# MaartenGr/ReinLife

Measured on AMD Instinct MI355X. Metric: agent-steps/sec (env.step + policy fwd), 30x30 grid, 100 agents, higher is better.
Workload: dtype f32-grade policy via block-scaled 2 x f16 split on v_mfma_f32_32x32x16_f16 (f32 accumulate) / int32+u8 world state / f64 rewards

## Files before the change

### reinlife_amd/csrc/rl_policy_dev.h

```cpp
#pragma once
#include "rl_common.h"

namespace {

typedef float f32x16 __attribute__((ext_vector_type(16)));
typedef float f32x4 __attribute__((ext_vector_type(4)));
typedef float f32x4u __attribute__((ext_vector_type(4), aligned(4)));
typedef float f32x2 __attribute__((ext_vector_type(2)));
typedef _Float16 f16x8 __attribute__((ext_vector_type(8)));
typedef const float __attribute__((address_space(1))) gfloat;
typedef const f32x4 __attribute__((address_space(1))) gf32x4;

constexpr int kInChunks = 10;
constexpr int kPlanes = 2;
constexpr int kScaleExp = 10;

__host__ __device__ constexpr int64_t frag_floats(int chunks, int tout) { return (int64_t)chunks * tout * kPlanes * 64 * 4; }
__host__ __device__ constexpr int64_t in_layer_floats(int tout) { return frag_floats(kInChunks, tout) + (int64_t)tout * 64; }
__host__ __device__ constexpr int64_t hid_layer_floats(int tin, int tout) { return frag_floats(2 * tin, tout) + (int64_t)tout * 64; }
__host__ __device__ constexpr int64_t head_consts_off(int tin) { return frag_floats(2 * tin, 1); }
__host__ __device__ constexpr int64_t head_floats(int tin, int nout) { return head_consts_off(tin) + 16; }

struct Layout {
    int64_t l1, l2a, l2b, ha, hb, total;
// ... 464 lines not shown
        a1 = mfma16(ac[1][0], B[S][1], a1); __builtin_amdgcn_sched_barrier(0);
    }
    a0 = mfma16(ac[0][0], B[S][0], a0); shadow(IntC<S>{}, IntC<0>{}, IntC<4 * S + 0>{}); __builtin_amdgcn_sched_barrier(0);
    a1 = mfma16(ac[1][0], B[S][0], a1); shadow(IntC<S>{}, IntC<1>{}, IntC<4 * S + 1>{}); __builtin_amdgcn_sched_barrier(0);
    a0 = mfma16(ac[0][1], B[S][0], a0); shadow(IntC<S>{}, IntC<2>{}, IntC<4 * S + 2>{}); __builtin_amdgcn_sched_barrier(0);
    a1 = mfma16(ac[1][1], B[S][0], a1); shadow(IntC<S>{}, IntC<3>{}, IntC<4 * S + 3>{}); __builtin_amdgcn_sched_barrier(0);
    if constexpr (S + 1 < kInChunks) k_pass_inx_steps<HALF, XM, S + 1>(w, B, a0, a1, shadow);
}
template <int HALF, int XM, typename Ring, typename Shadow>
__device__ __forceinline__ void k_pass_inx(Ring& w, const f32x4 (&B)[kInChunks][kPlanes], f32x16& a0, f32x16& a1, Shadow&& shadow)
{
#pragma unroll
    for (int r = 0; r < 16; ++r) { a0[r] = 0.0f; a1[r] = 0.0f; }
    k_pass_inx_steps<HALF, XM, 0>(w, B, a0, a1, shadow);
}
template <int XM, int C, int K, typename Raw>
__device__ __forceinline__ void in_split_slot(Raw&& raw, float sc, f32x4& hi, f32x4& lo)
{
    constexpr int cls = in_chunk_class(C);
    { float v; split_hi(raw(2 * K), raw(2 * K + 1), sc, v); hi[K] = v; }
    if constexpr (K == 1 || K == 3) {
        if constexpr (!(cls != 0 && XM >= cls)) {
            float v;
            split_lo(raw(2 * K - 2), raw(2 * K - 1), sc, hi[K - 1], v); lo[K - 1] = v;
            split_lo(raw(2 * K), raw(2 * K + 1), sc, hi[K], v); lo[K] = v;
        }
    }
}

template <int NS, int HALF, typename Ring, typename Shadow>
__device__ inline void k_pass(Ring& w, const f32x4 (&B)[NS][kPlanes], f32x16& a0, f32x16& a1, Shadow&& shadow)
{
#pragma unroll
    for (int r = 0; r < 16; ++r) { a0[r] = 0.0f; a1[r] = 0.0f; }
#pragma unroll
    for (int s = 0; s < NS; ++s) {
        f32x4 ac[2][kPlanes];
        w.take(HALF * NS + s, ac);
        a0 = mfma16(ac[0][0], B[s][1], a0); shadow(6 * s + 0); __builtin_amdgcn_sched_barrier(0);
        a1 = mfma16(ac[1][0], B[s][1], a1); shadow(6 * s + 1); __builtin_amdgcn_sched_barrier(0);
        a0 = mfma16(ac[0][0], B[s][0], a0); shadow(6 * s + 2); __builtin_amdgcn_sched_barrier(0);
        a1 = mfma16(ac[1][0], B[s][0], a1); shadow(6 * s + 3); __builtin_amdgcn_sched_barrier(0);
        a0 = mfma16(ac[0][1], B[s][0], a0); shadow(6 * s + 4); __builtin_amdgcn_sched_barrier(0);
        a1 = mfma16(ac[1][1], B[s][0], a1); shadow(6 * s + 5); __builtin_amdgcn_sched_barrier(0);
    }
}

__device__ inline void max3_abs(float& m, float a, float b)
{
#if defined(__HIP_DEVICE_COMPILE__)
    asm("v_max3_f32 %0, %0, |%1|, |%2|" : "+v"(m) : "v"(a), "v"(b));
#endif
}

struct EpiStream {
    const float* c;
    f32x4 un[2], bi[2];
    __device__ inline void fetch(int t, int Q)
    {
        const float* q = c + (t + (Q >> 2)) * 64 + 4 * (Q & 3);
        un[Q & 1] = *(const f32x4*)q;
        bi[Q & 1] = *(const f32x4*)(q + 16);
    }
    __device__ inline void step(int t, int e, f32x16& a0, f32x16& a1, float row_un, float& m)
    {
        const int Q = e >> 2, r = e & 15, ee = e & 3;
        if (ee == 0 && Q + 1 < 8) fetch(t, Q + 1);
        f32x16& a = e < 16 ? a0 : a1;
        const float y = fmaxf(__builtin_fmaf(a[r], un[Q & 1][ee] * row_un, bi[Q & 1][ee]), 0.0f);
        a[r] = y;
        m = fmaxf(m, y);
    }
};

template <int D, int NCH = 8, typename Raw>
__device__ inline void head_stream(WRing<1, 1, 1, D>& w, const f32x4& un4, Raw&& raw, float sc, float row_un, float (&out)[4])
{
    f32x16 a0, a1, a2;
#pragma unroll
    for (int r = 0; r < 16; ++r) { a0[r] = 0.0f; a1[r] = 0.0f; a2[r] = 0.0f; }
    f32x4 B[NCH][kPlanes];
#pragma unroll
    for (int k = 0; k < 3; ++k) split_slice<3>(k, [&](int e) { return raw(0, e); }, sc, B[0][0], B[0][1]);
#pragma unroll
    for (int s = 0; s < NCH; ++s) {
        f32x4 ac[1][kPlanes];
        w.template next<NCH>(s, ac);
        a0 = mfma16(ac[0][0], B[s][1], a0);
        if (s + 1 < NCH) split_slice<3>(0, [&](int e) { return raw(s + 1, e); }, sc, B[(s + 1) % NCH][0], B[(s + 1) % NCH][1]);
        __builtin_amdgcn_sched_barrier(0);
        a1 = mfma16(ac[0][0], B[s][0], a1);
        if (s + 1 < NCH) split_slice<3>(1, [&](int e) { return raw(s + 1, e); }, sc, B[(s + 1) % NCH][0], B[(s + 1) % NCH][1]);
        __builtin_amdgcn_sched_barrier(0);
        a2 = mfma16(ac[0][1], B[s][0], a2);
        if (s + 1 < NCH) split_slice<3>(2, [&](int e) { return raw(s + 1, e); }, sc, B[(s + 1) % NCH][0], B[(s + 1) % NCH][1]);
        __builtin_amdgcn_sched_barrier(0);
    }
#pragma unroll
    for (int r = 0; r < 4; ++r) out[r] = ((a0[r] + a1[r]) + a2[r]) * (un4[r] * row_un);
}

struct PairLds {
    float* pmax;
    f32x4* ex;
    float* val;
};
struct Tile1Part {
    float head[4];
    rl_u4 draw;
};

#ifndef RL_CERT_COUNT
#define RL_CERT_COUNT(greedy_mask, cert_mask, fell_back) do { } while (0)
#endif
template <int KIND>
__device__ __attribute__((noinline, cold)) void tile1_cert_fallback(TileIO io, const f32x4* ex, float un1, f32x4 adv4, rl_u4 draw)
{
    extern __shared__ __attribute__((aligned(16))) char rl_dyn_lds[];
    constexpr int D = 3;
    const int lane = (int)__builtin_amdgcn_mbcnt_hi(~0u, __builtin_amdgcn_mbcnt_lo(~0u, 0u)), h = lane >> 5;
    const Layout L = layout_of(KIND);
    const float* const consts = (const float*)(rl_dyn_lds + io.c_lds_off) + 32 * h;
    const float* const hconsts = (const float*)(rl_dyn_lds + io.c_lds_off) + 768;
    WRingH<8, D> w;
    w.start(io.packed + L.l2b, lane);
    f32x4 B2[8][kPlanes];
#pragma unroll
    for (int c = 0; c < 8; ++c)
#pragma unroll
        for (int pl = 0; pl < kPlanes; ++pl) B2[c][pl] = ex[(c * kPlanes + pl) * 64 + lane];
    f32x16 A[4];
    EpiStream ep;
    float mrow = 0.0f;
    k_pass<8, 0>(w, B2, A[0], A[1], [&](int) {});
    ep.c = consts + 512;
    k_pass<8, 1>(w, B2, A[2], A[3], [&](int slot) {
        if (slot == 0) ep.fetch(0, 0);
        if (slot >= 2 && slot < 34) ep.step(0, slot - 2, A[0], A[1], un1, mrow);
    });
    WRing<1, 1, 1, D> wh;
    wh.start(io.packed + L.hb, lane, 0);
    ep.fetch(2, 0);
#pragma unroll
    for (int e = 0; e < 32; ++e) ep.step(2, e, A[2], A[3], un1, mrow);
    mrow = fmaxf(mrow, __shfl_xor(mrow, 32));
    float sc2, un2;
    row_scale(mrow, sc2, un2);
    auto araw = [&](int c, int e) { return A[c >> 1][8 * (c & 1) + e]; };
    float val[4];
    head_stream<D>(wh, *(const f32x4*)(hconsts + 16 + 4 * h), araw, sc2, un2, val);
    const float adv[4] = {adv4.x, adv4.y, adv4.z, adv4.w};
    tile1_finish<KIND>(io, lane, adv, val[0] + hconsts[16 + 8], draw, *(const f32x4*)(hconsts + 8 + 4 * h));
}
template <int KIND>
__device__ inline void tile1_finish_cert(const TileIO& io, int lane, const float (&adv)[4], const rl_u4& draw, const float* hconsts, float vbar,
                                         const f32x4* ex, float un1)
{
    const int h = lane >> 5;
    const f32x4 ba = *(const f32x4*)(hconsts + 8 + 4 * h);
    const float a4[4] = {adv[0] + ba.x, adv[1] + ba.y, adv[2] + ba.z, adv[3] + ba.w};
    float o4[4];
#pragma unroll
    for (int r = 0; r < 4; ++r) o4[r] = __shfl_xor(a4[r], 32);
    int act = 0;
    bool greedy = false, ok = true;
    if (h == 0) {
        const float a[8] = {a4[0], a4[1], a4[2], a4[3], o4[0], o4[1], o4[2], o4[3]};
        float best = a[0], amax = fabsf(a[0]), s = a[0];
        int is = 0;
#pragma unroll
        for (int i = 1; i < 8; ++i) {
            const bool gt = a[i] > best;
            is = gt ? i : is; best = gt ? a[i] : best;
            amax = fmaxf(amax, fabsf(a[i])); s += a[i];
        }
        const float thr = 0x1p-20f * (((amax + amax) + vbar) + 0x1p-80f) + (s - s);
#pragma unroll
        for (int j = 0; j < 7; ++j) ok = ok && (j >= is || best - a[j] > thr);
        const bool explore = (float)rl_u24(draw.x) < io.eps;
        act = explore ? (int)(draw.y >> 29) : is;
        greedy = io.valid && io.actions && !explore;
    }
    const bool need = greedy && !ok;
    RL_CERT_COUNT(__ballot(greedy), __ballot(greedy && ok), __any(need));
    if (__builtin_expect(__any(need), 0)) {
        tile1_cert_fallback<KIND>(io, ex, un1, f32x4{adv[0], adv[1], adv[2], adv[3]}, draw);
        return;
    }
    if (h == 0 && io.valid && io.actions) {
        io.actions[io.row] = (int8_t)act;
        if (io.lds_actions_off >= 0) {
            extern __shared__ __attribute__((aligned(16))) char rl_dyn_lds[];
            ((signed char*)rl_dyn_lds)[io.lds_actions_off + io.lds_slot] = (signed char)act;
        }
    }
}

__device__ inline void cert_bound_part(gfloat* __restrict__ pk, int tid, double& c0, double& c1)
{
    const Layout L = layout_of(RL_PERD3QN);
    const int t2 = tid >> 7, pl = (tid >> 6) & 1, lane = tid & 63, oo = lane & 31, o = 32 * t2 + oo;
    const int h = (oo >> 2) & 1, r = (oo & 3) + 4 * (oo >> 3);
    gf32x4* f = (gf32x4*)(pk + L.l2b) + (t2 * kPlanes + pl) * 64 + lane;
    f32x4 u[8];
#pragma unroll
    for (int s = 0; s < 8; ++s) u[s] = f[s * 4 * kPlanes * 64];
    const float un_o = pk[L.l2b + frag_floats(8, 4) + (t2 * 2 + h) * 32 + r], b1 = pk[L.l2b + frag_floats(8, 4) + (t2 * 2 + h) * 32 + 16 + r];
    typedef const _Float16 __attribute__((address_space(1))) gf16;
    gf16* hw = (gf16*)(pk + L.hb);
    const int hidx = (((o >> 5) * 2 + (r >> 3)) * kPlanes * 64 + 32 * h) * 8 + (r & 7);
    const double w = (double)fabsf((float)hw[hidx]) + (double)fabsf((float)hw[hidx + 64 * 8]);
    const double un_v = (double)pk[L.hb + head_consts_off(4)];
    double sum = 0.0;
#pragma unroll
    for (int s = 0; s < 8; ++s) {
        const f16x8 v = __builtin_bit_cast(f16x8, u[s]);
#pragma unroll
        for (int e = 0; e < 8; ++e) sum += (double)fabsf((float)v[e]);
    }
    const double wv = w * un_v;
    c1 = wv * (sum * (double)un_o);
    c0 = (pl == 0 && lane < 32) ? wv * (double)fabsf(b1) : 0.0;
}
__device__ inline float f32_up(double d)
{
    float f = (float)d;
    if ((double)f < d) f = __builtin_bit_cast(float, __builtin_bit_cast(unsigned, f) + (f >= 0.0f ? 1u : -1u));
    return f;
}

template <int KIND, bool COHERENT, bool PAIR = false, int XM = 0, bool CERT = false>
__device__ inline void policy_tile1s(const TileIO& io, int lane, int role = 0, const PairLds* pair_lds = nullptr, Tile1Part* part = nullptr)
{
    static_assert(KIND == RL_D3QN || KIND == RL_PERD3QN, "one-wave tile: dueling kinds");
    static_assert(!CERT || PAIR, "the certified argmax: the pair tile");
    extern __shared__ __attribute__((aligned(16))) char rl_dyn_lds[];
    constexpr int D = 3;
    const int h = lane >> 5;
    const Layout L = layout_of(KIND);
    gfloat* __restrict__ packed = io.packed;
    const float* const consts = (const float*)(rl_dyn_lds + io.c_lds_off) + 32 * h;
    const float* const hconsts = (const float*)(rl_dyn_lds + io.c_lds_off) + 768;
    RL_PMARK1(1);
    WRingH<kInChunks, D, PAIR ? kInChunks : 2 * kInChunks> w1;
    w1.start(packed + L.l1 + (PAIR ? role * (2 * kPlanes * 64 * 4) : 0), lane);
    f32x4 X[kInChunks][2];
    {
        const int64_t rbase = io.row * RL_OBS_DIM;
        if (io.x_lds_off >= 0) {
            const float* xr = (const float*)(rl_dyn_lds + io.x_lds_off);
#pragma unroll
            for (int c = 0; c < kInChunks; ++c)
#pragma unroll
                for (int q = 0; q < 2; ++q) {
                    if (c == kInChunks - 1 && h == 1) X[c][q] = f32x4{xr[149], xr[150], xr[151], xr[152]};
                    else X[c][q] = *(const f32x4*)(xr + 16 * c + 8 * h + 4 * q);
                }
        } else
#pragma unroll
        for (int c = 0; c < kInChunks; ++c)
#pragma unroll
            for (int q = 0; q < 2; ++q) {
                const int k0 = (c == kInChunks - 1 && h == 1) ? 149 : 16 * c + 8 * h + 4 * q;
                if (COHERENT) {
                    const __amdgpu_buffer_rsrc_t rsrc = __builtin_amdgcn_make_buffer_rsrc((void*)io.obs, 0, 0x7fffffff, 0x00027000);
                    X[c][q] = __builtin_bit_cast(f32x4, __builtin_amdgcn_raw_buffer_load_b128(rsrc, (int)((rbase + k0) * 4), 0, 16 ));
                } else
                    X[c][q] = *(const f32x4u*)(io.obs + rbase + k0);
            }
    }
    rl_u4 draw = {0u, 0u, 0u, 0u};
    if ((!PAIR || role == 0) && io.actions && io.eps > 0.0f) draw = rl_philox4x32(io.seed, io.key_epoch, io.key_world, io.key_tick, RL_SITE_ACT, io.key_index);
    if (h == 1) { X[kInChunks - 1][0] = f32x4{X[kInChunks - 1][0].w, 0.0f, 0.0f, 0.0f}; X[kInChunks - 1][1] = f32x4{0.0f, 0.0f, 0.0f, 0.0f}; }
    float sc0, un0;
    if constexpr (XM >= 1) row_scale(1.0f, sc0, un0);
    else {
        float m4[4] = {0.0f, 0.0f, 0.0f, 0.0f};
#pragma unroll
        for (int c = 0; c < kInChunks; ++c)
#pragma unroll
            for (int q = 0; q < 2; ++q) {
                max3_abs(m4[(2 * c + q) & 3], X[c][q].x, X[c][q].y);
                max3_abs(m4[(2 * c + q + 2) & 3], X[c][q].z, X[c][q].w);
            }
        float m = fmaxf(fmaxf(m4[0], m4[1]), fmaxf(m4[2], m4[3]));
        m = fmaxf(m, __shfl_xor(m, 32));
        row_scale(m, sc0, un0);
    }
    f32x4 B1[kInChunks][kPlanes];
    auto xraw = [&](int c, int e) { return X[c][e >> 2][e & 3]; };
    f32x16 F[4];
    EpiStream ep;
    if constexpr (XM >= 1) {
        auto x0 = [&](int e) { return xraw(0, e); };
        in_split_slot<XM, 0, 0>(x0, sc0, B1[0][0], B1[0][1]); in_split_slot<XM, 0, 1>(x0, sc0, B1[0][0], B1[0][1]);
        in_split_slot<XM, 0, 2>(x0, sc0, B1[0][0], B1[0][1]); in_split_slot<XM, 0, 3>(x0, sc0, B1[0][0], B1[0][1]);
        RL_PMARK1(2);
        k_pass_inx<0, XM>(w1, B1, F[0], F[1], [&](auto st, auto k, auto) {
            constexpr int c = decltype(st)::value + 1;
            if constexpr (c < kInChunks) in_split_slot<XM, c, decltype(k)::value>([&](int e) { return xraw(c, e); }, sc0, B1[c][0], B1[c][1]);
        });
    } else {
#pragma unroll
        for (int k = 0; k < 6; ++k) split_slice<6>(k, [&](int e) { return xraw(0, e); }, sc0, B1[0][0], B1[0][1]);
        RL_PMARK1(2);
        k_pass<kInChunks, 0>(w1, B1, F[0], F[1], [&](int slot) {
            const int c = slot / 6 + 1;
            if (c < kInChunks) split_slice<6>(slot % 6, [&](int e) { return xraw(c, e); }, sc0, B1[c][0], B1[c][1]);
        });
    }
    float mrow = 0.0f;
    const int64_t l2 = (PAIR && role) ? L.l2b : L.l2a, hd = (PAIR && role) ? L.hb : L.ha;
    WRingH<8, D> w2;
    f32x4 B2[8][kPlanes];
    float sc1, un1;
    auto fraw = [&](int c, int e) { return F[c >> 1][8 * (c & 1) + e]; };
    [[maybe_unused]] float zrow = 0.0f;
    if (PAIR) {
        if (!(CERT && role)) w2.start(packed + l2, lane);
        ep.c = consts + role * 128;
        ep.fetch(0, 0);
#pragma unroll
        for (int e = 0; e < 32; ++e) ep.step(0, e, F[0], F[1], un0, mrow);
        mrow = fmaxf(mrow, __shfl_xor(mrow, 32));
        pair_lds->pmax[role * 64 + lane] = mrow;
        lds_barrier();
        mrow = fmaxf(mrow, pair_lds->pmax[(role ^ 1) * 64 + lane]);
        zrow = mrow;
        row_scale(mrow, sc1, un1);
#pragma unroll
        for (int c = 0; c < 4; ++c) {
            f32x4 hi, lo;
#pragma unroll
            for (int k = 0; k < 6; ++k) split_slice<6>(k, [&](int e) { return fraw(c, e); }, sc1, hi, lo);
            pair_lds->ex[((4 * role + c) * kPlanes + 0) * 64 + lane] = hi;
            pair_lds->ex[((4 * role + c) * kPlanes + 1) * 64 + lane] = lo;
        }
        lds_barrier();
        if (CERT && role) { RL_PMARK1(9); return; }
#pragma unroll
        for (int c = 0; c < 8; ++c)
#pragma unroll
            for (int pl = 0; pl < kPlanes; ++pl) B2[c][pl] = pair_lds->ex[(c * kPlanes + pl) * 64 + lane];
    } else {
        ep.c = consts;
        if constexpr (XM >= 1)
            k_pass_inx<1, XM>(w1, B1, F[2], F[3], [&](auto, auto, auto sl) {
                constexpr int slot = decltype(sl)::value;
                if constexpr (slot == 0) ep.fetch(0, 0);
                if constexpr (slot >= 2 && slot < 34) ep.step(0, slot - 2, F[0], F[1], un0, mrow);
            });
        else
        k_pass<kInChunks, 1>(w1, B1, F[2], F[3], [&](int slot) {
            if (slot == 0) ep.fetch(0, 0);
            if (slot >= 2 && slot < 34) ep.step(0, slot - 2, F[0], F[1], un0, mrow);
        });
        RL_PMARK1(3);
        w2.start(packed + l2, lane);
        ep.fetch(2, 0);
#pragma unroll
        for (int e = 0; e < 32; ++e) ep.step(2, e, F[2], F[3], un0, mrow);
        mrow = fmaxf(mrow, __shfl_xor(mrow, 32));
        row_scale(mrow, sc1, un1);
#pragma unroll
        for (int k = 0; k < 6; ++k) split_slice<6>(k, [&](int e) { return fraw(0, e); }, sc1, B2[0][0], B2[0][1]);
    }
    RL_PMARK1(4);
    f32x16 A[4];
    k_pass<8, 0>(w2, B2, A[0], A[1], [&](int slot) {
        const int c = slot / 6 + 1;
        if (!PAIR && c < 8) split_slice<6>(slot % 6, [&](int e) { return fraw(c, e); }, sc1, B2[c][0], B2[c][1]);
    });
    mrow = 0.0f;
    ep.c = consts + ((PAIR && role) ? 512 : 256);
    k_pass<8, 1>(w2, B2, A[2], A[3], [&](int slot) {
        if (slot == 0) ep.fetch(0, 0);
        if (slot >= 2 && slot < 34) ep.step(0, slot - 2, A[0], A[1], un1, mrow);
    });
    RL_PMARK1(5);
    WRing<1, 1, 1, D> wh;
    wh.start(packed + hd, lane, 0);
    ep.fetch(2, 0);
#pragma unroll
    for (int e = 0; e < 32; ++e) ep.step(2, e, A[2], A[3], un1, mrow);
    mrow = fmaxf(mrow, __shfl_xor(mrow, 32));
    float sc2, un2;
    row_scale(mrow, sc2, un2);
    auto araw = [&](int c, int e) { return A[c >> 1][8 * (c & 1) + e]; };
    float adv[4], val[4];
    RL_PMARK1(6);
    if (PAIR) {
        head_stream<D>(wh, *(const f32x4*)(hconsts + ((PAIR && role) ? 16 : 0) + 4 * h), araw, sc2, un2, adv);
        if constexpr (CERT) {
            const float* const kc = hconsts + kTileConstFloats - 768;
            tile1_finish_cert<KIND>(io, lane, adv, draw, hconsts, __builtin_fmaf(kc[1], zrow, kc[0]), pair_lds->ex, un1);
            RL_PMARK1(9);
            return;
        }
        if (role) { if (h == 0) pair_lds->val[lane] = adv[0] + hconsts[16 + 8]; }
        else {
#pragma unroll
            for (int r = 0; r < 4; ++r) part->head[r] = adv[r];
            part->draw = draw;
        }
        RL_PMARK1(9);
        return;
    }
    head_stream<D>(wh, *(const f32x4*)(hconsts + 4 * h), araw, sc2, un2, adv);
    WRingH<8, D> w3;
    w3.start(packed + L.l2b, lane);
    RL_PMARK1(7);
    k_pass<8, 0>(w3, B2, A[0], A[1], [&](int) {});
    mrow = 0.0f;
    ep.c = consts + 512;
    k_pass<8, 1>(w3, B2, A[2], A[3], [&](int slot) {
        if (slot == 0) ep.fetch(0, 0);
        if (slot >= 2 && slot < 34) ep.step(0, slot - 2, A[0], A[1], un1, mrow);
    });
    RL_PMARK1(8);
    wh.start(packed + L.hb, lane, 0);
    ep.fetch(2, 0);
#pragma unroll
    for (int e = 0; e < 32; ++e) ep.step(2, e, A[2], A[3], un1, mrow);
    mrow = fmaxf(mrow, __shfl_xor(mrow, 32));
    row_scale(mrow, sc2, un2);
    head_stream<D>(wh, *(const f32x4*)(hconsts + 16 + 4 * h), araw, sc2, un2, val);
    RL_PMARK1(9);
    tile1_finish<KIND>(io, lane, adv, val[0] + hconsts[16 + 8], draw, *(const f32x4*)(hconsts + 8 + 4 * h));
}


struct QuadLds {
    float* pmax;
    f32x4* ex;
    float* val;
#ifdef RL_PHASE_PROFILE
    long long* prof;
#endif
};
#ifdef RL_PHASE_PROFILE
#define RL_QMARK(pt) do { if (ql->prof && lane == 0) ql->prof[116 + 4 * (pt) + q] = (long long)clock64(); } while (0)
#else
#define RL_QMARK(pt) do { } while (0)
#endif
constexpr int kQuadExBytes = 24 * 1024;
constexpr int kQuadFloats = 3 * 32 * 4 + 32;
constexpr int kQuadBarriers = 6;

template <bool COHERENT, bool XL>
__device__ inline void quad_load_x(const TileIO& io, const float* xr, int goff, int c, int h, f32x4& x0, f32x4& x1)
{
    if (XL) {
        x0 = *(const f32x4*)(xr + 16 * c + 8 * h);
        x1 = *(const f32x4*)(xr + 16 * c + 8 * h + 4);
        return;
    }
    const bool last = c == kInChunks - 1 && h == 1;
    const int k0 = last ? 149 : 16 * c + 8 * h;
    if (COHERENT) {
        const __amdgpu_buffer_rsrc_t rsrc = __builtin_amdgcn_make_buffer_rsrc((void*)io.obs, 0, 0x7fffffff, 0x00027000);
        x0 = __builtin_bit_cast(f32x4, __builtin_amdgcn_raw_buffer_load_b128(rsrc, goff + 4 * k0, 0, 16 ));
        x1 = __builtin_bit_cast(f32x4, __builtin_amdgcn_raw_buffer_load_b128(rsrc, goff + 4 * (last ? k0 : k0 + 4), 0, 16));
    } else {
        const float* g = (const float*)((const char*)io.obs + goff);
        x0 = *(const f32x4u*)(g + k0);
        x1 = *(const f32x4u*)(g + (last ? k0 : k0 + 4));
    }
}
template <bool XL>
__device__ inline void quad_fix_x(int c, int h, f32x4& x0, f32x4& x1)
{
    if (!XL && c == kInChunks - 1 && h == 1) { x0 = f32x4{x0.w, 0.0f, 0.0f, 0.0f}; x1 = f32x4{0.0f, 0.0f, 0.0f, 0.0f}; }
}
__device__ inline float quad_row_max(const QuadLds* ql, int stage, int q, int lane, float m)
{
    m = fmaxf(m, __shfl_xor(m, 32));
    float* pm = ql->pmax + (stage * 32 + (lane & 31)) * 4;
    if (lane < 32) pm[q] = m;
    lds_barrier();
    const f32x4 v = *(const f32x4*)pm;
    return fmaxf(fmaxf(v.x, v.y), fmaxf(v.z, v.w));
}
template <int NS, int D, int TOUT = 4>
struct WRingQ {
    f32x4 a[D][kPlanes];
    gf32x4* p;
    __device__ inline void start(gfloat* __restrict__ pw, int lane, int tile)
    {
        p = (gf32x4*)pw + tile * kPlanes * 64 + lane;
#pragma unroll
        for (int d = 0; d < D; ++d)
#pragma unroll
            for (int pl = 0; pl < kPlanes; ++pl) a[d][pl] = p[(d * TOUT * kPlanes + pl) * 64];
        p += D * TOUT * kPlanes * 64;
        asm volatile("" : "+v"(p));
    }
    __device__ inline void take(int i, f32x4 (&ac)[kPlanes])
    {
        const int cur = i % D;
#pragma unroll
        for (int pl = 0; pl < kPlanes; ++pl) ac[pl] = a[cur][pl];
        if (i + D < NS) {
#ifdef RL_ABL_HALFW
            a[cur][0] = p[0]; a[cur][1] = a[cur][0];
#else
#pragma unroll
            for (int pl = 0; pl < kPlanes; ++pl) a[cur][pl] = p[pl * 64];
#endif
            p += TOUT * kPlanes * 64;
            asm volatile("" : "+v"(p));
        }
    }
};
__device__ inline float quad_epilogue(f32x16& a, const float* c, float row_un)
{
    float m = 0.0f;
#pragma unroll
    for (int Q = 0; Q < 4; ++Q) {
        const f32x4 un = *(const f32x4*)(c + 4 * Q), bi = *(const f32x4*)(c + 16 + 4 * Q);
#pragma unroll
        for (int e = 0; e < 4; ++e) {
            const float y = fmaxf(__builtin_fmaf(a[4 * Q + e], un[e] * row_un, bi[e]), 0.0f);
            a[4 * Q + e] = y;
            m = fmaxf(m, y);
        }
    }
    return m;
}
template <int Q, int D>
__device__ inline void quad_head(gfloat* __restrict__ hw, int lane, const f32x4 (&own)[2][kPlanes], const f32x4* __restrict__ others, const f32x4& un4, float row_un, float (&out)[4])
{
    WRing<1, 1, 1, D> w;
    w.start(hw, lane, 0);
    f32x16 a0, a1, a2;
#pragma unroll
    for (int r = 0; r < 16; ++r) { a0[r] = 0.0f; a1[r] = 0.0f; a2[r] = 0.0f; }
    auto src = [&](int c, int pl) -> f32x4 {
        const int wv = c >> 1;
        if (wv == Q) return own[c & 1][pl];
        const int idx = Q == 0 ? wv - 1 : (wv == 0 ? 0 : wv - 1);
        return others[((idx * 2 + (c & 1)) * kPlanes + pl) * 64 + lane];
    };
    f32x4 B[2][kPlanes];
#pragma unroll
    for (int pl = 0; pl < kPlanes; ++pl) B[0][pl] = src(0, pl);
#pragma unroll
    for (int s = 0; s < 8; ++s) {
        f32x4 ac[1][kPlanes];
        w.template next<8>(s, ac);
        if (s + 1 < 8) {
#pragma unroll
            for (int pl = 0; pl < kPlanes; ++pl) B[(s + 1) & 1][pl] = src(s + 1, pl);
        }
        a0 = mfma16(ac[0][0], B[s & 1][1], a0);
        a1 = mfma16(ac[0][0], B[s & 1][0], a1);
        a2 = mfma16(ac[0][1], B[s & 1][0], a2);
        __builtin_amdgcn_sched_barrier(0);
    }
#pragma unroll
    for (int r = 0; r < 4; ++r) out[r] = ((a0[r] + a1[r]) + a2[r]) * (un4[r] * row_un);
}

template <int KIND, bool COHERENT, bool XL>
__device__ inline void quad_input_layer(const TileIO& io, int lane, int q, const QuadLds* ql, rl_u4& draw, f32x16& F, float& un0)
{
    extern __shared__ __attribute__((aligned(16))) char rl_dyn_lds[];
    const int h = lane >> 5;
    const Layout L = layout_of(KIND);
    const float* const xr = (const float*)(rl_dyn_lds + (XL ? io.x_lds_off : 0));
    const int goff = XL ? 0 : (int)(io.row * (RL_OBS_DIM * 4));
    f32x4 X[3][2];
#pragma unroll
    for (int i = 0; i < 3; ++i) {
        const int c = q + 4 * i;
        if (c < kInChunks) { quad_load_x<COHERENT, XL>(io, xr, goff, c, h, X[i][0], X[i][1]); quad_fix_x<XL>(c, h, X[i][0], X[i][1]); }
        else { X[i][0] = f32x4{0.0f, 0.0f, 0.0f, 0.0f}; X[i][1] = f32x4{0.0f, 0.0f, 0.0f, 0.0f}; }
    }
    WRingQ<kInChunks, 4> w1;
    w1.start(io.packed + L.l1, lane, q);
    if (q == 0 && io.actions && io.eps > 0.0f) draw = rl_philox4x32(io.seed, io.key_epoch, io.key_world, io.key_tick, RL_SITE_ACT, io.key_index);
    float m4[4] = {0.0f, 0.0f, 0.0f, 0.0f};
// ... 811 lines not shown
```

### reinlife_amd/csrc/rl_run.hip

```cpp
#include <mutex>
#include "rl_world_dev.h"
#ifndef RL_XM_DUELING_KERNEL
#define RL_XM_DUELING_KERNEL 0
#endif
#if RL_XM_DUELING_KERNEL != 0 && !defined(RL_XM_SELF_GENERATED_STATES_ONLY)
#error "RL_XM_DUELING_KERNEL != 0 is valid for self-generated states only: add -DRL_XM_SELF_GENERATED_STATES_ONLY to an A/B build that knows"
#endif
#ifndef RL_XM_ALL_DUELING_TILE
#define RL_XM_ALL_DUELING_TILE RL_XM_ALL_KERNEL
#endif
#ifndef RL_CERT_ALL
#define RL_CERT_ALL 0
#endif
#ifndef RL_XM_ALL_KERNEL
#define RL_XM_ALL_KERNEL 2
#endif

#ifdef RL_TUNING
#if !(defined(RL_RUN_UNIT) && RL_RUN_UNIT == 1)
static int g_run_debug = 0;
extern "C" __attribute__((visibility("default"))) void rl_debug_set_run_mask(int mask) { g_run_debug = mask; }
extern "C" __attribute__((visibility("default"))) int rl_debug_get_run_mask(void) { return g_run_debug; }
#endif
#define RL_RUN_DBG(ka) (*(const int __attribute__((address_space(4)))*)&(ka)->ra.debug)
// ... 156 lines not shown
        s.pos[tid] = r_pos; s.health[tid] = r_h; s.age[tid] = r_age; s.max_age[tid] = r_ma; s.gene[tid] = r_g; s.brain[tid] = r_b;
        s.uid[tid] = r_u; s.flags[tid] = r_fl; s.fitness[tid] = r_f;
        if (!open) s.action[tid] = r_act;
        s.aux[tid] = 0; s.src[tid] = (short)tid; s.order[tid] = (short)tid; s.newidx[tid] = (short)tid;
        s.occ[(r_pos & 255) * p.W + (r_pos >> 8)] = (short)tid;
    }
    for (int c = tid; c < p.Cp; c += T) ((unsigned*)s.foodv)[c] = 0u;
    for (int i = tid; i < p.hash_size; i += T) { s.hkey[i] = -1; s.hcnt[i] = 0u; }
    if (tid < RL_MAX_BRAINS) s.present[tid] = 0;
    if (SPEC) for (int i = tid; i < 2 * p.cap; i += T) ((unsigned*)s.reward)[i] = 0u;
    if (tid < S_COUNT)
        s.scal[tid] = tid == S_NSLOTS ? n : tid == S_TICK ? tick : tid == S_EPOCH ? epoch : tid == S_NEXT_UID ? next_uid : tid == S_MAX_GENE ? max_gene : 0;
    const bool drain = drain_stores || (also_drain && __builtin_amdgcn_readfirstlane(*also_drain) != 0);
    if (drain) asm volatile("s_waitcnt vmcnt(0)" ::: "memory");
    if (!open || drain) lds_barrier();
}

struct RunParams {
    KParams p;
    RunArgs ra;
};
template <int TRAIN>
__device__ inline float run_eps(RunParamsC* ka, int b, int n_brains, const PolSmem& ps)
{
    typedef const float __attribute__((address_space(4))) cfloat;
    if (TRAIN) {
        if (*(const int __attribute__((address_space(4)))*)&ka->ra.eps_inline_on)
            return ((cfloat*)ka->ra.eps_inline)[__builtin_amdgcn_readfirstlane(ps.meta[3]) * n_brains + b];
        const float* es = *(const float* const __attribute__((address_space(4)))*)&ka->ra.eps_sched;
        if (es) return ((cfloat*)es)[__builtin_amdgcn_readfirstlane(ps.meta[3]) * n_brains + b];
    }
    return ((cfloat*)ka->ra.eps)[b];
}

__host__ __device__ constexpr int run_plane_stride(int T, int W, int H) { return T >= 512 ? plane_stride(W, H) : W; }
template <bool FIXED, int T>
__device__ inline KParams run_params(RunParamsC* ka)
{
#if defined(__HIP_DEVICE_COMPILE__)
    KParams p = *(const KParams __attribute__((address_space(4)))*)&ka->p;
#else
    KParams p{};
#endif
    if (FIXED) {
        p.W = kFixW; p.H = kFixH; p.C = kFixC; p.Cp = kFixCp; p.nW = kFixCp / 64; p.PS = run_plane_stride(T, kFixW, kFixH); p.invW = kFixInvW;
        p.cap = kFixCap; p.hash_size = kFixHash; p.hash_mask = kFixHash - 1;
    }
    return p;
}
constexpr size_t kRunLdsBudget = 160 * 1024;
__host__ __device__ constexpr size_t run_mirror_budget(int T) { return T >= 512 ? kRunLdsBudget : 0; }
__host__ __device__ constexpr int run_cbrains(int T, int n_brains) { return T >= 512 ? n_brains : 0; }
template <int KIND> __host__ __device__ constexpr int run_tile_floats(int T) { return T == 1024 ? kQuadFloats : run_pair_floats<KIND>(); }
__host__ __device__ constexpr size_t run_min_region(int T) { return T == 1024 ? 4 * (size_t)kQuadExBytes : 0; }
template <bool FIXED, int KIND>
__device__ inline void run_carve(const KParams& p, Smem& s, PolSmem& ps, char* smem_raw, int T)
{
    const size_t o0 = FIXED ? carve(s, smem_raw, kFixCp, kFixCap, kFixHash, plane_words(run_plane_stride(T, kFixW, kFixH), kFixH, kFixCp))
                            : carve(s, smem_raw, p.Cp, p.cap, p.hash_size, plane_words(p.PS, p.H, p.Cp));
    carve_policy<KIND>(ps, smem_raw, o0, p.cap, run_mirror_budget(T), run_cbrains(T, p.n_brains), run_tile_floats<KIND>(T), run_min_region(T));
}

template <typename F>
__device__ inline void policy_lists_wave0(const KParams& p, PolSmem& ps, int n, int lane, F brain_of)
{
    if (lane < p.n_brains) ps.bcnt[lane] = 0;
    for (int base = 0; base < n; base += 64) {
        const int k = base + lane;
        if (k < n) {
            const int b = brain_of(k);
            const int pos = __hip_atomic_fetch_add(&ps.bcnt[b], 1, __ATOMIC_RELAXED, __HIP_MEMORY_SCOPE_WORKGROUP);
            ps.prow[k] = (short)(unsigned short)(pos | (b << 10));
        }
    }
    const int mine = lane < p.n_brains ? ps.bcnt[lane] : 0;
    const int tiles = (mine + 31) >> 5;
    const int tincl = wave_incl_scan(tiles);
    const int first_tile = tincl - tiles;
    if (lane < p.n_brains) ps.tstart[lane] = first_tile;
    if (lane == 63) ps.meta[0] = tincl;
    const int tt = min(read_lane(tincl, 63), kMaxTiles);
    for (int e = lane; e < tt * 32; e += 64) ps.trow[e] = (short)0x8000;
    if (lane < tt) {
        int b = 0;
        for (int bb = 1; bb < p.n_brains; ++bb) if (read_lane(first_tile, bb) <= lane && read_lane(mine, bb) > 0) b = bb;
        ps.tbrain[lane] = b;
    }
    for (int base = 0; base < n; base += 64) {
        const int k = base + lane;
        if (k < n) {
            const int e = (unsigned short)ps.prow[k], pos = e & 1023, b = e >> 10;
            const int t = ps.tstart[b] + (pos >> 5);
            if (t < kMaxTiles) ps.trow[t * 32 + (pos & 31)] = (short)k;
        }
    }
}

__device__ inline int run_obs_flags(const KParams& p, const Smem& s, int n, int bad_health)
{
    if (bad_health || n >= 2 * p.max_agents) return 0;
    return RL_XF_SCALE | (s.type[0] == RL_AGENT ? 0 : RL_XF_INT_HEALTH);
}

__device__ inline void policy_schedule_wave0(const KParams& p, PolSmem& ps, RunParamsC* ka, int lane, bool first_call = false)
{
    const int nt = __builtin_amdgcn_readfirstlane(ps.meta[0]);
    const int t = lane & 3;
    const int brain = ps.tbrain[t] & (kRunMaxBrains - 1);
    const int kind = ps.bkind[brain];
    const int cost = t < nt ? (kind == RL_PPO ? 672 : kind == RL_DQN ? 180 : 360) : 0;
    const int ex = t < nt ? pair_ex_bytes(kind) : 0;
    int rank = 0, off = 0, total_ex = 0;
#pragma unroll
    for (int u = 0; u < 4; ++u) {
        const int cu = __builtin_amdgcn_readlane(cost, u), eu = __builtin_amdgcn_readlane(ex, u);
        rank += (cu > cost || (cu == cost && u < t)) ? 1 : 0;
        off += u < t ? eu : 0;
        total_ex += eu;
    }
    const size_t mirror_bytes = (size_t)ps.xrows * kXStride * sizeof(float);
    const bool pair_ok = nt <= 4 && ps.xmirror != nullptr && ps.pairv != nullptr && (size_t)total_ex <= mirror_bytes;
    const int fit = (int)(mirror_bytes / (size_t)pair_ex_bytes(RL_PPO));
    const int want = (0x22331100 >> (4 * (lane & 7))) & 15;
    int tile = -1, tb = 0, tk = 0;
#pragma unroll
    for (int u = 0; u < 4; ++u) {
        const int bu = __builtin_amdgcn_readlane(brain, u), ku = __builtin_amdgcn_readlane(kind, u);
        if (u < nt && __builtin_amdgcn_readlane(rank, u) == want) { tile = u; tb = bu; tk = ku; }
    }
    if (lane < 4) ps.texoff[lane] = off;
    if (lane < 8) ps.wtask[lane] = (pair_ok && tile >= 0) ? (tile | ((lane & 1) << 8) | (tb << 12) | (tk << 20)) : -1;
    if (lane == 0) {
        ps.meta[5] = pair_ok ? 0 : 1;
        if (first_call) ps.meta[6] = fit < 1 ? 1 : (fit > 4 ? 4 : fit);
    }
}

template <int T, int KIND, int TRAIN>
__device__ __forceinline__ void run_policy1(const KParams& p, Smem& s, PolSmem& ps, RunParamsC* ka, int w, int n, const float* obs_rows, char* smem_base, int wave)
{
    const int lane = rl_lane_fresh(), j = lane & 31;
    [[maybe_unused]] const int tid = wave * 64 + lane;
#ifdef RL_PHASE_PROFILE
    const long long t_entry = (long long)clock64();
#endif
    int ntiles = __builtin_amdgcn_readfirstlane(ps.meta[0]);
    {
        const int dbg = RL_RUN_DBG(ka);
        if (dbg & 4) ntiles = min(ntiles, 2);
        if (dbg & 8) ntiles = min(ntiles, 1);
        if (dbg & 16) ntiles = min(ntiles, 3);
    }
    const bool mirrored = ps.xmirror != nullptr && __builtin_amdgcn_readfirstlane(ps.meta[4]) != 0;
    auto tile_io = [&](int ti, TileIO& io, int j) {
        const int b = __builtin_amdgcn_readfirstlane(ps.tbrain[ti]);
        const int e = (unsigned short)ps.trow[ti * 32 + j], k = e & 0x7fff;
        io.packed = (gfloat*)((const float* const __attribute__((address_space(4)))*)ka->ra.packed)[b];
        io.obs = obs_rows;
        io.row = (int64_t)w * p.cap + k;
        io.valid = !(e & 0x8000);
        io.eps = run_eps<TRAIN>(ka, b, p.n_brains, ps);
        io.out = TRAIN == 2 ? *(float* const __attribute__((address_space(4)))*)&ka->ra.policy_out : nullptr;
        io.actions = *(int8_t* const __attribute__((address_space(4)))*)&ka->ra.actions;
        io.seed = p.seed;
        io.key_world = (uint32_t)(p.world_base + w); io.key_tick = (uint32_t)s.scal[S_TICK]; io.key_epoch = (uint32_t)s.scal[S_EPOCH];
        io.key_index = (uint32_t)k;
        io.lds_actions_off = (int)((char*)s.action - smem_base); io.lds_slot = k;
        io.x_lds_off = (mirrored && k < ps.xrows) ? (int)((char*)(ps.xmirror + k * kXStride) - smem_base) : -1;
        io.c_lds_off = ps.cconst ? (int)((char*)(ps.cconst + run_const_floats<KIND>() * b) - smem_base) : -1;
#ifdef RL_PHASE_PROFILE
        io.prof = (p.prof && (int)blockIdx.x == p.prof_world && wave == 0) ? p.prof : nullptr;
        if (io.prof && lane == 0) { io.prof[100] = t_entry; io.prof[110] = (long long)clock64(); }
#endif
    };
    if constexpr (T == 1024) {
        const int q = __builtin_amdgcn_readfirstlane(wave >> 2), slot = wave & 3;
        for (int t0 = 0; t0 < ntiles; t0 += 4) {
            const int lane = rl_lane_fresh(), j = lane & 31;
            const int ti = t0 + slot;
            const bool have = ti < ntiles;
            TileIO io;
            Tile1Part part;
            QuadLds ql;
            ql.pmax = ps.pairv + kQuadFloats * slot; ql.val = ql.pmax + 3 * 32 * 4;
            ql.ex = (f32x4*)((char*)ps.xmirror + (size_t)kQuadExBytes * slot);
#ifdef RL_PHASE_PROFILE
            ql.prof = (p.prof && (int)blockIdx.x == p.prof_world && slot == 0) ? p.prof : nullptr;
#endif
            if (have) {
                tile_io(ti, io, j);
                if (ntiles > 4) io.x_lds_off = -1;
                policy_quad<KIND, RL_RUN_COHERENT>(io, lane, q, &ql, &part);
            } else {
#pragma unroll
                for (int i = 0; i < kQuadBarriers; ++i) lds_barrier();
            }
            lds_barrier();
            if (have && q == 0) tile1_finish<KIND>(io, lane, part.head, ql.val[j], part.draw, *(const f32x4*)((const float*)(smem_base + io.c_lds_off) + 768 + 8 + 4 * (lane >> 5)));
        }
    } else
    if (T == 512 && ps.pairv != nullptr && ntiles <= 4 && (size_t)ps.xrows * kXStride * sizeof(float) >= 4 * (size_t)kPairExBytes) {
        const int role = __builtin_amdgcn_readfirstlane(wave >> 2), slot = wave & 3;
        const bool have = slot < ntiles;
        const bool cert = TRAIN != 2 && !(RL_RUN_DBG(ka) & 64);
        TileIO io;
        Tile1Part part;
        PairLds pl;
        pl.val = ps.pairv + kPairFloats * slot; pl.pmax = pl.val + 32;
        pl.ex = (f32x4*)((char*)ps.xmirror + (size_t)kPairExBytes * slot);
        if (have) {
            tile_io(slot, io, j);
            if (cert) policy_tile1s<KIND, RL_RUN_COHERENT, true, RL_XM_DUELING_KERNEL, TRAIN != 2>(io, lane, role, &pl, &part);
            else policy_tile1s<KIND, RL_RUN_COHERENT, true, RL_XM_DUELING_KERNEL>(io, lane, role, &pl, &part);
        } else { lds_barrier(); lds_barrier(); }
#ifdef RL_PHASE_PROFILE
        if (p.prof && (int)blockIdx.x == p.prof_world && lane == 0) p.prof[116 + wave] = (long long)clock64();
#endif
        if (!cert) {
            lds_barrier();
            if (have && role == 0) {
                const int fl = rl_lane_fresh();
                tile1_finish<KIND>(io, fl, part.head, pl.val[fl & 31], part.draw, *(const f32x4*)((const float*)(smem_base + io.c_lds_off) + 768 + 8 + 4 * (fl >> 5)));
            }
        }
    } else
    for (int ti = wave; ti < ntiles; ti += T / 64) {
        TileIO io;
        tile_io(ti, io, j);
        if (T == 512) policy_tile1s<KIND, RL_RUN_COHERENT, false, RL_XM_DUELING_KERNEL>(io, lane);
        else policy_tile1<KIND, RL_RUN_COHERENT, true>(io, lane);
    }
#ifdef RL_PHASE_PROFILE
    if (p.prof && (int)blockIdx.x == p.prof_world && tid == 0) p.prof[111] = (long long)clock64();
#endif
    lds_barrier();
#ifdef RL_PHASE_PROFILE
    if (p.prof && (int)blockIdx.x == p.prof_world && tid == 0) p.prof[112] = (long long)clock64();
#endif
}

#ifndef RL_XM_COLD_CALL
#define RL_XM_COLD_CALL 0
#endif
#ifndef RL_XM_LIKELY
#define RL_XM_LIKELY 1
#endif
#if RL_XM_LIKELY
#define RL_XM_EXPECT(x) __builtin_expect_with_probability(!!(x), 1, 0.9)
#else
#define RL_XM_EXPECT(x) (x)
#endif
template <bool CERT>
__device__ __attribute__((noinline, cold)) Tile1Part run_tile_general(TileIO io, PairLds pl, int role, int kind)
{
    Tile1Part part;
    const int lane = rl_lane_fresh();
    if (kind == RL_DQN) policy_pair2<RL_DQN, RL_RUN_COHERENT>(io, lane, role, &pl, &part);
    else if (kind == RL_PPO) policy_pair2<RL_PPO, RL_RUN_COHERENT>(io, lane, role, &pl, &part);
    else policy_tile1s<RL_PERD3QN, RL_RUN_COHERENT, true, 0, CERT>(io, lane, role, &pl, &part);
    return part;
}

template <int T, int TRAIN>
__device__ __forceinline__ void run_policy_all(const KParams& p, Smem& s, PolSmem& ps, RunParamsC* ka, int w, int n, const float* obs_rows, char* smem_base, int wave)
{
    static_assert(T == 512, "kKindAll: 512-thread workgroups");
    typedef const int __attribute__((address_space(4))) cint;
    const int lane = rl_lane_fresh(), j = lane & 31;
#ifdef RL_PHASE_PROFILE
    if (p.prof && (int)blockIdx.x == p.prof_world && wave == 0 && lane == 0) p.prof[100] = (long long)clock64();
#endif
    const int ntiles = __builtin_amdgcn_readfirstlane(ps.meta[0]);
    const bool mirrored = ps.xmirror != nullptr && __builtin_amdgcn_readfirstlane(ps.meta[4]) != 0;
    const bool fallback = __builtin_amdgcn_readfirstlane(ps.meta[5]) != 0;
    constexpr int xneed = RL_XM_ALL_KERNEL == 2 ? (RL_XF_SCALE | RL_XF_INT_HEALTH) : RL_XF_SCALE;
#ifdef RL_XM_ASSUME_ALWAYS
    const bool rows_known = true;
#else
    const bool rows_known = RL_XM_ALL_KERNEL != 0 && (__builtin_amdgcn_readfirstlane(ps.oflags[0]) & xneed) == xneed;
#endif
    auto tile_io = [&](int ti, TileIO& io, bool from_mirror, int task) {
        const int b = task >= 0 ? ((task >> 12) & 255) : __builtin_amdgcn_readfirstlane(ps.tbrain[ti]);
        const int e = (unsigned short)ps.trow[ti * 32 + j], k = e & 0x7fff;
        io.packed = (gfloat*)((const float* const __attribute__((address_space(4)))*)ka->ra.packed)[b];
        io.obs = obs_rows;
        io.row = (int64_t)w * p.cap + k;
        io.valid = !(e & 0x8000);
        io.eps = run_eps<TRAIN>(ka, b, p.n_brains, ps);
        io.out = TRAIN == 2 ? *(float* const __attribute__((address_space(4)))*)&ka->ra.policy_out : nullptr;
        io.actions = *(int8_t* const __attribute__((address_space(4)))*)&ka->ra.actions;
        io.seed = p.seed;
        io.key_world = (uint32_t)(p.world_base + w); io.key_tick = (uint32_t)s.scal[S_TICK]; io.key_epoch = (uint32_t)s.scal[S_EPOCH];
        io.key_index = (uint32_t)k;
        io.lds_actions_off = (int)((char*)s.action - smem_base); io.lds_slot = k;
        io.x_lds_off = (from_mirror && mirrored && k < ps.xrows) ? (int)((char*)(ps.xmirror + k * kXStride) - smem_base) : -1;
        io.c_lds_off = (int)((char*)(ps.cconst + kTileConstMax * b) - smem_base);
#ifdef RL_PHASE_PROFILE
        io.prof = (p.prof && (int)blockIdx.x == p.prof_world && wave == ((p.ablate >> 20) & 7)) ? p.prof : nullptr;
#endif
        return task >= 0 ? ((task >> 20) & 7) : ((cint*)ka->ra.kind)[b];
    };
    const bool cert = RL_CERT_ALL && TRAIN != 2 && !(RL_RUN_DBG(ka) & 64);
    auto duel = [&](auto xm, TileIO& io, int role, PairLds& pl, Tile1Part& part) {
        if (cert) policy_tile1s<RL_PERD3QN, RL_RUN_COHERENT, true, decltype(xm)::value, TRAIN != 2>(io, lane, role, &pl, &part);
        else policy_tile1s<RL_PERD3QN, RL_RUN_COHERENT, true, decltype(xm)::value>(io, lane, role, &pl, &part);
    };
    auto pair_round = [&](bool have, int ti, int role, int slot, int ex_off, bool from_mirror, int task) {
        TileIO io;
        Tile1Part part;
        PairLds pl;
        int kind = -1;
        if (have) {
            kind = __builtin_amdgcn_readfirstlane(tile_io(ti, io, from_mirror, task));
            pl.val = ps.pairv + kPairFloatsAll * slot; pl.pmax = pl.val + kPairValFloats;
            pl.ex = (f32x4*)((char*)ps.xmirror + ex_off);
            const bool plain = kind == RL_DQN || kind == RL_PPO;
            if (!plain && RL_XM_ALL_DUELING_TILE == 0) duel(IntC<0>{}, io, role, pl, part);
            else if (RL_XM_EXPECT(rows_known)) {
                if (kind == RL_DQN) policy_pair2<RL_DQN, RL_RUN_COHERENT, RL_XM_ALL_KERNEL>(io, lane, role, &pl, &part);
                else if (kind == RL_PPO) policy_pair2<RL_PPO, RL_RUN_COHERENT, RL_XM_ALL_KERNEL>(io, lane, role, &pl, &part);
                else duel(IntC<RL_XM_ALL_DUELING_TILE>{}, io, role, pl, part);
            } else if (RL_XM_COLD_CALL) part = cert ? run_tile_general<TRAIN != 2>(io, pl, role, kind) : run_tile_general<false>(io, pl, role, kind);
            else {
                if (kind == RL_DQN) policy_pair2<RL_DQN, RL_RUN_COHERENT>(io, lane, role, &pl, &part);
                else if (kind == RL_PPO) policy_pair2<RL_PPO, RL_RUN_COHERENT>(io, lane, role, &pl, &part);
                else duel(IntC<0>{}, io, role, pl, part);
            }
        } else { lds_barrier(); lds_barrier(); }
        lds_barrier();
        if (have && role == 0) {
            const int fl = rl_lane_fresh();
            if (kind == RL_DQN) pair_finish<RL_DQN>(io, fl, part, &pl);
            else if (kind == RL_PPO) pair_finish<RL_PPO>(io, fl, part, &pl);
            else if (!cert) tile1_finish<RL_PERD3QN>(io, fl, part.head, pl.val[fl & 31], part.draw, *(const f32x4*)((const float*)(smem_base + io.c_lds_off) + 768 + 8 + 4 * (fl >> 5)));
        }
    };
    const int pr = __builtin_amdgcn_readfirstlane(ps.meta[6]);
    const int task = __builtin_amdgcn_readfirstlane(ps.wtask[wave]);
    const int n_rounds = fallback ? (ntiles + pr - 1) / pr : 1;
    for (int r = 0; r < n_rounds; ++r) {
        const int slot = fallback ? (wave & 3) : (task & 255);
        const int ti = fallback ? r * pr + slot : slot;
        const bool have = fallback ? (slot < pr && ti < ntiles) : task >= 0;
        const int role = __builtin_amdgcn_readfirstlane(fallback ? (wave >> 2) : ((task >> 8) & 1));
        const int ex_off = fallback ? slot * pair_ex_bytes(RL_PPO) : (have ? ps.texoff[slot] : 0);
        pair_round(have, ti, role, slot, ex_off, !fallback, fallback ? -1 : task);
        if (fallback) lds_barrier();
    }
#ifdef RL_PHASE_PROFILE
    if (p.prof && (int)blockIdx.x == p.prof_world && lane == 0) p.prof[116 + wave] = (long long)clock64();
    if (p.prof && (int)blockIdx.x == p.prof_world && wave == 0 && lane == 0) p.prof[111] = (long long)clock64();
#endif
    lds_barrier();
#ifdef RL_PHASE_PROFILE
    if (p.prof && (int)blockIdx.x == p.prof_world && wave == 0 && lane == 0) p.prof[112] = (long long)clock64();
#endif
}

template <int T, bool FIXED, int KIND, int TRAIN>
__device__ __forceinline__ void run_policy_half(RunParamsC* ka, int wave)
{
    extern __shared__ __attribute__((aligned(16))) char smem_raw[];
    const KParams p = run_params<FIXED, T>(ka);
    Smem s;
    PolSmem ps;
    run_carve<FIXED, KIND>(p, s, ps, smem_raw, T);
    const int w = blockIdx.x;
    const int n = __builtin_amdgcn_readfirstlane(ps.meta[1]), cur = __builtin_amdgcn_readfirstlane(ps.meta[2]);
    const float* obs_in = ((float* const __attribute__((address_space(4)))*)ka->ra.obs)[cur];
    if constexpr (KIND == kKindAll) run_policy_all<T, TRAIN>(p, s, ps, ka, w, n, obs_in, smem_raw, wave);
    else run_policy1<T, KIND, TRAIN>(p, s, ps, ka, w, n, obs_in, smem_raw, wave);
}

template <int T>
__device__ inline void patch_planes_after_update(const KParams& p, Smem& s, int n1, int first_new, int end_new)
{
    const int tid = rl_tidx();
    bool cell0 = false;
    for (int k = tid; k < n1; k += T) {
        const int a = s.order[k];
        const int fl = s.flags[a], ps = s.pos[a];
        if (fl & RL_F_DEAD) {
            const int c = (ps & 255) * p.PS + (ps >> 8);
// ... 654 lines not shown
```

Before: 1.075 billion.

## Use certified argmax in single-wave tile path, skipping value head

```diff
diff --git a/reinlife_amd/csrc/rl_policy_dev.h b/reinlife_amd/csrc/rl_policy_dev.h
--- a/reinlife_amd/csrc/rl_policy_dev.h
+++ b/reinlife_amd/csrc/rl_policy_dev.h
@@ -640,9 +640,9 @@
     const float adv[4] = {adv4.x, adv4.y, adv4.z, adv4.w};
     tile1_finish<KIND>(io, lane, adv, val[0] + hconsts[16 + 8], draw, *(const f32x4*)(hconsts + 8 + 4 * h));
 }
-template <int KIND>
+template <int KIND, typename Fallback>
 __device__ inline void tile1_finish_cert(const TileIO& io, int lane, const float (&adv)[4], const rl_u4& draw, const float* hconsts, float vbar,
-                                         const f32x4* ex, float un1)
+                                         Fallback&& fallback)
 {
     const int h = lane >> 5;
     const f32x4 ba = *(const f32x4*)(hconsts + 8 + 4 * h);
@@ -672,7 +672,7 @@
     const bool need = greedy && !ok;
     RL_CERT_COUNT(__ballot(greedy), __ballot(greedy && ok), __any(need));
     if (__builtin_expect(__any(need), 0)) {
-        tile1_cert_fallback<KIND>(io, ex, un1, f32x4{adv[0], adv[1], adv[2], adv[3]}, draw);
+        fallback();
         return;
     }
     if (h == 0 && io.valid && io.actions) {
@@ -717,11 +717,13 @@
     return f;
 }
 
+template <int KIND, bool COHERENT, int XM>
+__device__ __attribute__((noinline, cold)) void tile1s_full_cold(TileIO io);
+
 template <int KIND, bool COHERENT, bool PAIR = false, int XM = 0, bool CERT = false>
 __device__ inline void policy_tile1s(const TileIO& io, int lane, int role = 0, const PairLds* pair_lds = nullptr, Tile1Part* part = nullptr)
 {
     static_assert(KIND == RL_D3QN || KIND == RL_PERD3QN, "one-wave tile: dueling kinds");
-    static_assert(!CERT || PAIR, "the certified argmax: the pair tile");
     extern __shared__ __attribute__((aligned(16))) char rl_dyn_lds[];
     constexpr int D = 3;
     const int h = lane >> 5;
@@ -849,6 +851,7 @@
 #pragma unroll
         for (int e = 0; e < 32; ++e) ep.step(2, e, F[2], F[3], un0, mrow);
         mrow = fmaxf(mrow, __shfl_xor(mrow, 32));
+        zrow = mrow;
         row_scale(mrow, sc1, un1);
 #pragma unroll
         for (int k = 0; k < 6; ++k) split_slice<6>(k, [&](int e) { return fraw(0, e); }, sc1, B2[0][0], B2[0][1]);
@@ -881,7 +884,8 @@
         head_stream<D>(wh, *(const f32x4*)(hconsts + ((PAIR && role) ? 16 : 0) + 4 * h), araw, sc2, un2, adv);
         if constexpr (CERT) {
             const float* const kc = hconsts + kTileConstFloats - 768;
-            tile1_finish_cert<KIND>(io, lane, adv, draw, hconsts, __builtin_fmaf(kc[1], zrow, kc[0]), pair_lds->ex, un1);
+            tile1_finish_cert<KIND>(io, lane, adv, draw, hconsts, __builtin_fmaf(kc[1], zrow, kc[0]),
+                                    [&]() { tile1_cert_fallback<KIND>(io, pair_lds->ex, un1, f32x4{adv[0], adv[1], adv[2], adv[3]}, draw); });
             RL_PMARK1(9);
             return;
         }
@@ -895,6 +899,12 @@
         return;
     }
     head_stream<D>(wh, *(const f32x4*)(hconsts + 4 * h), araw, sc2, un2, adv);
+    if constexpr (CERT) {
+        const float* const kc = hconsts + kTileConstFloats - 768;
+        tile1_finish_cert<KIND>(io, lane, adv, draw, hconsts, __builtin_fmaf(kc[1], zrow, kc[0]), [&]() { tile1s_full_cold<KIND, COHERENT, XM>(io); });
+        RL_PMARK1(9);
+        return;
+    }
     WRingH<8, D> w3;
     w3.start(packed + L.l2b, lane);
     RL_PMARK1(7);
@@ -915,6 +925,12 @@
     head_stream<D>(wh, *(const f32x4*)(hconsts + 16 + 4 * h), araw, sc2, un2, val);
     RL_PMARK1(9);
     tile1_finish<KIND>(io, lane, adv, val[0] + hconsts[16 + 8], draw, *(const f32x4*)(hconsts + 8 + 4 * h));
+}
+template <int KIND, bool COHERENT, int XM>
+__device__ __attribute__((noinline, cold)) void tile1s_full_cold(TileIO io)
+{
+    const int lane = (int)__builtin_amdgcn_mbcnt_hi(~0u, __builtin_amdgcn_mbcnt_lo(~0u, 0u));
+    policy_tile1s<KIND, COHERENT, false, XM, false>(io, lane);
 }
 
 
diff --git a/reinlife_amd/csrc/rl_run.hip b/reinlife_amd/csrc/rl_run.hip
--- a/reinlife_amd/csrc/rl_run.hip
+++ b/reinlife_amd/csrc/rl_run.hip
@@ -332,6 +332,7 @@
         if (dbg & 16) ntiles = min(ntiles, 3);
     }
     const bool mirrored = ps.xmirror != nullptr && __builtin_amdgcn_readfirstlane(ps.meta[4]) != 0;
+    [[maybe_unused]] const bool cert = T == 512 && TRAIN != 2 && !(RL_RUN_DBG(ka) & 64);
     auto tile_io = [&](int ti, TileIO& io, int j) {
         const int b = __builtin_amdgcn_readfirstlane(ps.tbrain[ti]);
         const int e = (unsigned short)ps.trow[ti * 32 + j], k = e & 0x7fff;
@@ -379,10 +380,9 @@
             if (have && q == 0) tile1_finish<KIND>(io, lane, part.head, ql.val[j], part.draw, *(const f32x4*)((const float*)(smem_base + io.c_lds_off) + 768 + 8 + 4 * (lane >> 5)));
         }
     } else
-    if (T == 512 && ps.pairv != nullptr && ntiles <= 4 && (size_t)ps.xrows * kXStride * sizeof(float) >= 4 * (size_t)kPairExBytes) {
+    if (T == 512 && !cert && ps.pairv != nullptr && ntiles <= 4 && (size_t)ps.xrows * kXStride * sizeof(float) >= 4 * (size_t)kPairExBytes) {
         const int role = __builtin_amdgcn_readfirstlane(wave >> 2), slot = wave & 3;
         const bool have = slot < ntiles;
-        const bool cert = TRAIN != 2 && !(RL_RUN_DBG(ka) & 64);
         TileIO io;
         Tile1Part part;
         PairLds pl;
@@ -390,25 +390,27 @@
         pl.ex = (f32x4*)((char*)ps.xmirror + (size_t)kPairExBytes * slot);
         if (have) {
             tile_io(slot, io, j);
-            if (cert) policy_tile1s<KIND, RL_RUN_COHERENT, true, RL_XM_DUELING_KERNEL, TRAIN != 2>(io, lane, role, &pl, &part);
-            else policy_tile1s<KIND, RL_RUN_COHERENT, true, RL_XM_DUELING_KERNEL>(io, lane, role, &pl, &part);
+            policy_tile1s<KIND, RL_RUN_COHERENT, true, RL_XM_DUELING_KERNEL>(io, lane, role, &pl, &part);
         } else { lds_barrier(); lds_barrier(); }
 #ifdef RL_PHASE_PROFILE
         if (p.prof && (int)blockIdx.x == p.prof_world && lane == 0) p.prof[116 + wave] = (long long)clock64();
 #endif
-        if (!cert) {
-            lds_barrier();
-            if (have && role == 0) {
-                const int fl = rl_lane_fresh();
-                tile1_finish<KIND>(io, fl, part.head, pl.val[fl & 31], part.draw, *(const f32x4*)((const float*)(smem_base + io.c_lds_off) + 768 + 8 + 4 * (fl >> 5)));
-            }
-        }
-    } else
-    for (int ti = wave; ti < ntiles; ti += T / 64) {
-        TileIO io;
-        tile_io(ti, io, j);
-        if (T == 512) policy_tile1s<KIND, RL_RUN_COHERENT, false, RL_XM_DUELING_KERNEL>(io, lane);
-        else policy_tile1<KIND, RL_RUN_COHERENT, true>(io, lane);
+        lds_barrier();
+        if (have && role == 0) {
+            const int fl = rl_lane_fresh();
+            tile1_finish<KIND>(io, fl, part.head, pl.val[fl & 31], part.draw, *(const f32x4*)((const float*)(smem_base + io.c_lds_off) + 768 + 8 + 4 * (fl >> 5)));
+        }
+    } else {
+        for (int ti = wave; ti < ntiles; ti += T / 64) {
+            TileIO io;
+            tile_io(ti, io, j);
+            if (T == 512 && cert) policy_tile1s<KIND, RL_RUN_COHERENT, false, RL_XM_DUELING_KERNEL, T == 512 && TRAIN != 2>(io, lane);
+            else if (T == 512) policy_tile1s<KIND, RL_RUN_COHERENT, false, RL_XM_DUELING_KERNEL>(io, lane);
+            else policy_tile1<KIND, RL_RUN_COHERENT, true>(io, lane);
+        }
+#ifdef RL_PHASE_PROFILE
+        if (T == 512 && p.prof && (int)blockIdx.x == p.prof_world && lane == 0) p.prof[116 + wave] = (long long)clock64();
+#endif
     }
 #ifdef RL_PHASE_PROFILE
     if (p.prof && (int)blockIdx.x == p.prof_world && tid == 0) p.prof[111] = (long long)clock64();
```

Measured after the change: 1.097 billion, median of 6. +2.0%, better.
